# hruffieux/atlasqtl

Measured on NVIDIA B200. Metric: SNPxtrait CAVI updates/s, higher is better.
Workload: dtype f64

## Files before the change

### atlasqtl_b200/_lib.py

```python
import ctypes
import os

import numpy as np

_HERE = os.path.dirname(os.path.abspath(__file__))
LIB_PATH = os.environ.get("AQ_LIB") or os.path.join(_HERE, "libatlasqtl_b200.so")
_DP = ctypes.POINTER(ctypes.c_double)
_IP = ctypes.POINTER(ctypes.c_int32)

EXPORTS = ["aq_last_error", "aq_version", "aq_device_info", "aq_create", "aq_destroy", "aq_dims", "aq_set_order",
           "aq_set_state", "aq_get_state", "aq_get_residual", "aq_refresh_tables", "aq_sweep", "aq_rowsums_zpart",
           "aq_rowsums_zpart_dev", "aq_launch_count", "aq_last_sweep_ms", "aq_last_ms", "aq_sync", "aq_coreDualLoop",
           "aq_set_missing", "aq_set_state_mis", "aq_sweep_mis", "aq_ppi_count_sum", "aq_ppi_next_above", "aq_ppi_collect",
           "aq_prep_x", "aq_prep_geno", "aq_prep_result", "aq_prep_destroy", "aq_prep_launch_count", "aq_create_prepared",
           "aq_get_x", "aq_get_y", "aq_snapshot", "aq_snapshot_fetch", "aq_coreDualMisLoop", "aq_sweep_plan",
           "aq_test_logistic", "aq_prep_dims", "aq_release_x"]


class AtlasqtlB200Error(RuntimeError):
    pass


_lib = None


def load():
    global _lib
    if _lib is not None:
        return _lib
    if not os.path.exists(LIB_PATH):
        raise AtlasqtlB200Error(f"{LIB_PATH} not found: build it with `python -m atlasqtl_b200.build` "
                                "(there is no CPU fallback for the CAVI sweep)")
    lib = ctypes.CDLL(LIB_PATH)
    lib.aq_last_error.restype = ctypes.c_char_p
    lib.aq_launch_count.restype = ctypes.c_int64
    lib.aq_launch_count.argtypes = [ctypes.c_void_p]
    lib.aq_prep_launch_count.restype = ctypes.c_int64
    lib.aq_prep_launch_count.argtypes = [ctypes.c_void_p]
    _lib = lib
    return lib


def check(rc):
    if rc != 0:
        raise AtlasqtlB200Error(f"atlasqtl_b200 error {rc}: {load().aq_last_error().decode()}")


def dptr(a):
    if a is None:
        return None
    assert isinstance(a, np.ndarray) and a.dtype == np.float64
    return a.ctypes.data_as(_DP)


def iptr(a):
    if a is None:
        return None
    assert isinstance(a, np.ndarray) and a.dtype == np.int32 and a.flags.c_contiguous
    return a.ctypes.data_as(_IP)


def fmat(a):
    return np.asfortranarray(a, dtype=np.float64)
```

### atlasqtl_b200/compat.py

```python
import ctypes

import numpy as np

from . import _lib


def coreDualLoop(cp_X, cp_Y_X, gam_vb, log_Phi_theta_plus_zeta, log_1_min_Phi_theta_plus_zeta, log_sig2_inv_vb,
                 log_tau_vb, m1_beta, cp_betaX_X, mu_beta_vb, sig2_beta_vb, tau_vb, shuffled_ind, sample_q, c=1.0,
                 device=0):
    lib = _lib.load()
    p, q = gam_vb.shape
    mats = (cp_X, cp_Y_X, gam_vb, log_Phi_theta_plus_zeta, log_1_min_Phi_theta_plus_zeta, m1_beta, cp_betaX_X, mu_beta_vb)
    for m in mats:
        if not (isinstance(m, np.ndarray) and m.dtype == np.float64 and m.flags.f_contiguous):
            raise TypeError("matrices must be Fortran-ordered float64 arrays (R's double storage)")
    if cp_X.shape != (p, p) or cp_Y_X.shape != (q, p):
        raise ValueError("cp_X must be p x p and cp_Y_X q x p")
    vecs = [np.ascontiguousarray(v, dtype=np.float64) for v in (log_tau_vb, sig2_beta_vb, tau_vb)]
    si = np.ascontiguousarray(shuffled_ind, dtype=np.int32)
    sq = np.ascontiguousarray(sample_q, dtype=np.int32)
    _lib.check(lib.aq_coreDualLoop(ctypes.c_int(device), p, q, _lib.dptr(cp_X), _lib.dptr(cp_Y_X), _lib.dptr(gam_vb),
                                   _lib.dptr(log_Phi_theta_plus_zeta), _lib.dptr(log_1_min_Phi_theta_plus_zeta),
                                   ctypes.c_double(log_sig2_inv_vb), _lib.dptr(vecs[0]), _lib.dptr(m1_beta),
                                   _lib.dptr(cp_betaX_X), _lib.dptr(mu_beta_vb), _lib.dptr(vecs[1]), _lib.dptr(vecs[2]),
                                   _lib.iptr(si), len(si), _lib.iptr(sq), len(sq), ctypes.c_double(c)))


def coreDualMisLoop(cp_X, cp_X_rm, cp_Y_X, gam_vb, log_Phi_theta_plus_zeta, log_1_min_Phi_theta_plus_zeta, log_sig2_inv_vb,
                    log_tau_vb, m1_beta, cp_betaX_X, mu_beta_vb, sig2_beta_vb, tau_vb, shuffled_ind, sample_q, c=1.0,
                    device=0):
    lib = _lib.load()
    p, q = gam_vb.shape
    mats = (cp_X, cp_Y_X, gam_vb, log_Phi_theta_plus_zeta, log_1_min_Phi_theta_plus_zeta, m1_beta, cp_betaX_X, mu_beta_vb,
            sig2_beta_vb) + tuple(cp_X_rm)
    for m in mats:
        if not (isinstance(m, np.ndarray) and m.dtype == np.float64 and m.flags.f_contiguous):
            raise TypeError("matrices must be Fortran-ordered float64 arrays (R's double storage)")
    if cp_X.shape != (p, p) or cp_Y_X.shape != (q, p) or sig2_beta_vb.shape != (p, q):
        raise ValueError("cp_X must be p x p, cp_Y_X q x p and sig2_beta_vb p x q")
    if len(cp_X_rm) != q or any(m.shape != (p, p) for m in cp_X_rm):
        raise ValueError("cp_X_rm must be a list of q p x p matrices")
    vecs = [np.ascontiguousarray(v, dtype=np.float64) for v in (log_tau_vb, tau_vb)]
    si = np.ascontiguousarray(shuffled_ind, dtype=np.int32)
    sq = np.ascontiguousarray(sample_q, dtype=np.int32)
    rm = (_lib._DP * q)(*[_lib.dptr(m) for m in cp_X_rm])
    _lib.check(lib.aq_coreDualMisLoop(ctypes.c_int(device), p, q, _lib.dptr(cp_X), rm, _lib.dptr(cp_Y_X), _lib.dptr(gam_vb),
                                      _lib.dptr(log_Phi_theta_plus_zeta), _lib.dptr(log_1_min_Phi_theta_plus_zeta),
                                      ctypes.c_double(log_sig2_inv_vb), _lib.dptr(vecs[0]), _lib.dptr(m1_beta),
                                      _lib.dptr(cp_betaX_X), _lib.dptr(mu_beta_vb), _lib.dptr(sig2_beta_vb),
                                      _lib.dptr(vecs[1]), _lib.iptr(si), len(si), _lib.iptr(sq), len(sq),
                                      ctypes.c_double(c)))


def logistic_neg_device(x, device=0, variant=0):
    lib = _lib.load()
    x = np.ascontiguousarray(x, dtype=np.float64)
    out = np.empty_like(x)
    _lib.check(lib.aq_test_logistic(ctypes.c_int(device), ctypes.c_int(variant), _lib.dptr(x), _lib.dptr(out),
                                    ctypes.c_int(x.size)))
    return out
```

### atlasqtl_b200/csrc/aq_api.cu

```cuda
#include <algorithm>
#include <cmath>
#include <cstdio>
#include <cstdlib>
#include <cstring>
#include <numeric>
#include <string>
#include <vector>

#include "../../include/atlasqtl_b200.h"
#include "aq_internal.h"
#include "aq_mis.cuh"
#include "aq_prep.cuh"
#include "aq_select.cuh"
#include "aq_stream.cuh"
#include "aq_sweep.cuh"

using namespace aq;

namespace {

thread_local std::string g_err;

int fail(int code, const std::string& msg) {
    g_err = msg;
// ... 536 lines not shown
    if (c->stream) cudaStreamSynchronize(c->stream);
    double* bufs[] = {c->xraw, c->xtiles, c->ymat, c->resid, c->gam, c->mu, c->dtab, c->wtab, c->i0tab, c->tvec,
                      c->ovec, c->theta, c->zeta, c->rowsum, c->partials, c->scalar, c->stage};
    for (double* b : bufs)
        if (b) cudaFree(b);
    if (c->order_dev) cudaFree(c->order_dev);
    if (c->seg_done) cudaFree(c->seg_done);
    if (c->mask) cudaFree(c->mask);
    if (c->mbits) cudaFree(c->mbits);
    if (c->mis_off_dev) cudaFree(c->mis_off_dev);
    if (c->mis_idx_dev) cudaFree(c->mis_idx_dev);
    for (double* b : {c->gk, c->atab, c->ltab})
        if (b) cudaFree(b);
    if (c->copy_stream) cudaStreamSynchronize(c->copy_stream);
    for (double* b : {c->sig2tab, c->xnsq, c->n_obs, c->mis_out, c->sel_partial, c->rowpart, c->snap_gam, c->snap_mu, c->stage2})
        if (b) cudaFree(b);
    if (c->ev0) cudaEventDestroy(c->ev0);
    if (c->ev1) cudaEventDestroy(c->ev1);
    for (cudaEvent_t e : {c->evr0, c->evr1, c->evt0, c->evt1})
        if (e) cudaEventDestroy(e);
    if (c->ev_snap) cudaEventDestroy(c->ev_snap);
    if (c->copy_stream) cudaStreamDestroy(c->copy_stream);
    if (c->stream) cudaStreamDestroy(c->stream);
    delete c;
    return AQ_OK;
}

}

namespace {
int create_impl(aq_ctx** out, int device, int n, int p, int q_local, const double* X, const aq_prep* prep, const double* Y,
                double* n_obs) {
    if (n < 2 || p < 1 || q_local < 1) return fail(AQ_EINVAL, "aq_create: need n >= 2, p >= 1, q >= 1");
    int sm = 0;
    int rc = aq_device_info(device, &sm, nullptr, nullptr);
    if (rc != AQ_OK) return rc;
    CfgInfo cfg;
    if (!pick_cfg(n, q_local, sm, &cfg))
        return fail(AQ_EUNSUPPORTED, "aq_create: n > 7168 is beyond the 8-CTA sample-split cluster kernel");
    aq_ctx* c = new aq_ctx();
    c->device = device;
    c->n = n;
    c->p = p;
    c->q = q_local;
    c->cfg = cfg;
    c->sm_count = sm;
    c->p_pad = (p + kBlk - 1) / kBlk * kBlk;
    c->q_pad = (q_local + 95) / 96 * 96;
    c->nb = c->p_pad / kBlk;
    c->ld_resid = cfg.n_pad * cfg.ncta;
    c->ntiles = (q_local + cfg.kT - 1) / cfg.kT;
    const size_t pq = (size_t)c->p_pad * c->q_pad;
    c->stage_cols = (int)std::max<size_t>(1, std::min<size_t>((size_t)q_local, ((size_t)256 << 20) / (sizeof(double) * (size_t)p)));
    c->n_partials = (size_t)((c->q + 255) / 256) * ((c->p + kTabRowsPerBlock - 1) / kTabRowsPerBlock);
#define AQ_ALLOC(ptr, count)                                                              \
    do {                                                                                  \
        cudaError_t e_ = cudaMalloc((void**)&(ptr), sizeof(*(ptr)) * (size_t)(count));    \
        if (e_ != cudaSuccess) {                                                          \
            cudaGetLastError();                                                           \
            aq_destroy(c);                                                                \
            return fail(AQ_ENOMEM, std::string("cudaMalloc ") + #ptr + ": " + cudaGetErrorString(e_)); \
        }                                                                                 \
    } while (0)
    AQ_ALLOC(c->xraw, (size_t)n * p);
    AQ_ALLOC(c->xtiles, (size_t)c->nb * cfg.ncta * cfg.tile_doubles);
    AQ_ALLOC(c->ymat, (size_t)c->q_pad * c->ld_resid);
    AQ_ALLOC(c->resid, (size_t)c->q_pad * c->ld_resid);
    AQ_ALLOC(c->gam, pq);
    AQ_ALLOC(c->mu, pq);
    AQ_ALLOC(c->dtab, pq);
    AQ_ALLOC(c->wtab, pq);
    AQ_ALLOC(c->i0tab, pq);
    AQ_ALLOC(c->tvec, 3 * (size_t)c->q_pad);
    AQ_ALLOC(c->ovec, 5 * (size_t)c->q_pad);
    AQ_ALLOC(c->theta, c->p_pad);
    AQ_ALLOC(c->zeta, c->q_pad);
    AQ_ALLOC(c->rowsum, c->p_pad);
    AQ_ALLOC(c->partials, c->n_partials);
    AQ_ALLOC(c->scalar, 8);
    AQ_ALLOC(c->stage, (size_t)c->stage_cols * p);
    AQ_ALLOC(c->order_dev, c->p_pad);
#undef AQ_ALLOC
    cudaError_t e = cudaStreamCreateWithFlags(&c->stream, cudaStreamNonBlocking);
    if (e == cudaSuccess) e = cudaEventCreate(&c->ev0);
    if (e == cudaSuccess) e = cudaEventCreate(&c->ev1);
    if (e == cudaSuccess) e = cudaEventCreate(&c->evr0);
    if (e == cudaSuccess) e = cudaEventCreate(&c->evr1);
    if (e == cudaSuccess) e = cudaEventCreate(&c->evt0);
    if (e == cudaSuccess) e = cudaEventCreate(&c->evt1);
    if (e == cudaSuccess) e = cudaMemsetAsync(c->ymat, 0, sizeof(double) * (size_t)c->q_pad * c->ld_resid, c->stream);
    if (e == cudaSuccess) e = cudaMemsetAsync(c->gam, 0, sizeof(double) * pq, c->stream);
    if (e == cudaSuccess) e = cudaMemsetAsync(c->mu, 0, sizeof(double) * pq, c->stream);
    if (e == cudaSuccess) e = cudaMemsetAsync(c->dtab, 0, sizeof(double) * pq, c->stream);
    if (e == cudaSuccess) e = cudaMemsetAsync(c->wtab, 0, sizeof(double) * pq, c->stream);
    if (e == cudaSuccess) e = cudaMemsetAsync(c->i0tab, 0, sizeof(double) * pq, c->stream);
    if (e == cudaSuccess) e = cudaMemsetAsync(c->ovec, 0, sizeof(double) * 5 * (size_t)c->q_pad, c->stream);
    if (e == cudaSuccess) e = cudaMemsetAsync(c->rowsum, 0, sizeof(double) * c->p_pad, c->stream);
    if (e == cudaSuccess && X) e = cudaMemcpyAsync(c->xraw, X, sizeof(double) * (size_t)n * p, cudaMemcpyHostToDevice, c->stream);
    if (e == cudaSuccess && prep) {
        if (prep->geno)
            materialise_kernel<<<p, 256, 0, c->stream>>>(SrcGeno{prep->gd, prep->bytes_per_col}, n, prep->st, prep->kept_dev, p, c->xraw);
        else
            materialise_kernel<<<p, 256, 0, c->stream>>>(SrcDouble{prep->xd, n}, n, prep->st, prep->kept_dev, p, c->xraw);
        e = cudaGetLastError();
        c->launches++;
    }
    if (e == cudaSuccess)
// ... 336 lines not shown
}

int aq_snapshot(aq_ctx* c) {
    if (!c) return fail(AQ_EINVAL, "NULL context");
    if (!c->have_state) return fail(AQ_ESTATE, "aq_snapshot before aq_set_state");
    AQ_CUDA(cudaSetDevice(c->device));
    const size_t pq = (size_t)c->p_pad * c->q_pad;
    if (!c->snap_gam) AQ_CUDA(cudaMalloc((void**)&c->snap_gam, sizeof(double) * pq));
    if (!c->snap_mu) AQ_CUDA(cudaMalloc((void**)&c->snap_mu, sizeof(double) * pq));
    if (!c->stage2) AQ_CUDA(cudaMalloc((void**)&c->stage2, sizeof(double) * (size_t)c->stage_cols * c->p));
    if (!c->ev_snap) AQ_CUDA(cudaEventCreateWithFlags(&c->ev_snap, cudaEventDisableTiming));
    if (!c->copy_stream) AQ_CUDA(cudaStreamCreateWithFlags(&c->copy_stream, cudaStreamNonBlocking));
    AQ_CUDA(cudaStreamSynchronize(c->copy_stream));
    AQ_CUDA(cudaMemcpyAsync(c->snap_gam, c->gam, sizeof(double) * pq, cudaMemcpyDeviceToDevice, c->stream));
    AQ_CUDA(cudaMemcpyAsync(c->snap_mu, c->mu, sizeof(double) * pq, cudaMemcpyDeviceToDevice, c->stream));
    AQ_CUDA(cudaEventRecord(c->ev_snap, c->stream));
    c->have_snap = true;
    return AQ_OK;
}

int aq_snapshot_fetch(aq_ctx* c, double* gam_vb, double* mu_beta_vb, double* beta_vb) {
    if (!c) return fail(AQ_EINVAL, "NULL context");
    if (!c->have_snap) return fail(AQ_ESTATE, "aq_snapshot_fetch before aq_snapshot");
    AQ_CUDA(cudaSetDevice(c->device));
    AQ_CUDA(cudaStreamWaitEvent(c->copy_stream, c->ev_snap, 0));
    double* outs[3] = {gam_vb, mu_beta_vb, beta_vb};
    for (int which = 0; which < 3; ++which) {
        if (!outs[which]) continue;
        const double* a = which == 1 ? c->snap_mu : c->snap_gam;
        const double* b = which == 2 ? c->snap_mu : nullptr;
        for (int k0 = 0; k0 < c->q; k0 += c->stage_cols) {
            const int kc = std::min(c->stage_cols, c->q - k0);
            dim3 grid((c->p + 31) / 32, (kc + 31) / 32), block(32, 8);
            dev_to_cm_kernel<<<grid, block, 0, c->copy_stream>>>(a, b, which == 2 ? 1 : 0, c->p, kc, k0, c->q_pad, c->stage2);
            AQ_CUDA(cudaGetLastError());
            AQ_CUDA(cudaMemcpyAsync(outs[which] + (size_t)k0 * c->p, c->stage2, sizeof(double) * (size_t)kc * c->p,
                                    cudaMemcpyDeviceToHost, c->copy_stream));
            AQ_CUDA(cudaStreamSynchronize(c->copy_stream));
        }
    }
    return AQ_OK;
}

int aq_get_residual(aq_ctx* c, double* resid) {
    if (!c || !resid) return fail(AQ_EINVAL, "NULL argument");
    if (!c->have_state) return fail(AQ_ESTATE, "aq_get_residual before aq_set_state");
    AQ_CUDA(cudaSetDevice(c->device));
    AQ_CUDA(cudaMemcpy2DAsync(resid, sizeof(double) * c->n, c->resid, sizeof(double) * c->ld_resid, sizeof(double) * c->n,
                              c->q, cudaMemcpyDeviceToHost, c->stream));
    AQ_CUDA(cudaStreamSynchronize(c->stream));
    return AQ_OK;
}

int aq_refresh_tables(aq_ctx* c, const double* theta_vb, const double* zeta_vb, double c_next, double* elbo_b_part) {
    if (!c || !theta_vb || !zeta_vb) return fail(AQ_EINVAL, "aq_refresh_tables: NULL argument");
    if (!(c_next > 0.0)) return fail(AQ_EINVAL, "aq_refresh_tables: c_next must be positive");
    if (elbo_b_part && !c->have_state) return fail(AQ_ESTATE, "aq_refresh_tables: ELBO part needs a state");
    AQ_CUDA(cudaSetDevice(c->device));
    c->rowpart_rows = 0;
    AQ_CUDA(cudaMemcpyAsync(c->theta, theta_vb, sizeof(double) * c->p, cudaMemcpyHostToDevice, c->stream));
    AQ_CUDA(cudaMemcpyAsync(c->zeta, zeta_vb, sizeof(double) * c->q, cudaMemcpyHostToDevice, c->stream));
    const int c_is_one = std::fabs(c_next - 1.0) < 1.5e-8;
    dim3 grid((c->q + 255) / 256, (c->p + kTabRowsPerBlock - 1) / kTabRowsPerBlock);
    AQ_CUDA(cudaEventRecord(c->evt0, c->stream));
    tables_kernel<<<grid, 256, 0, c->stream>>>(c->theta, c->zeta, c->p, c->q, c->q_pad, c_is_one ? 1.0 : std::sqrt(c_next),
                                               c_is_one, c->gam, c->dtab, c->wtab, c->i0tab, elbo_b_part ? 1 : 0,
                                               c->partials);
    AQ_CUDA(cudaGetLastError());
    c->launches++;
    if (elbo_b_part) {
        sum_partials_kernel<<<1, 1024, 0, c->stream>>>(c->partials, c->n_partials, c->scalar);
        AQ_CUDA(cudaGetLastError());
        c->launches++;
        AQ_CUDA(cudaMemcpyAsync(elbo_b_part, c->scalar, sizeof(double), cudaMemcpyDeviceToHost, c->stream));
    }
    AQ_CUDA(cudaEventRecord(c->evt1, c->stream));
    AQ_CUDA(cudaStreamSynchronize(c->stream));
    AQ_CUDA(cudaEventElapsedTime(&c->last_tables_ms, c->evt0, c->evt1));
    c->have_tables = true;
    return AQ_OK;
}

int aq_sweep(aq_ctx* c, double cc, double log_sig2_inv_vb, const double* tau_vb, const double* log_tau_vb,
             const double* sig2_beta_vb, double* colsum_gam, double* colsum_gam_mu2, double* colsum_beta2,
             double* resid_sq, double* colsum_zpart) {
    if (!c || !tau_vb || !log_tau_vb || !sig2_beta_vb) return fail(AQ_EINVAL, "aq_sweep: NULL argument");
    if (c->has_mis) return fail(AQ_ESTATE, "aq_sweep: this context has missing responses, use aq_sweep_mis");
    if (!c->have_state) return fail(AQ_ESTATE, "aq_sweep before aq_set_state");
    if (!c->have_tables) return fail(AQ_ESTATE, "aq_sweep before aq_refresh_tables");
    if (!(cc > 0.0)) return fail(AQ_EINVAL, "aq_sweep: c must be positive");
    AQ_CUDA(cudaSetDevice(c->device));
    AQ_CUDA(cudaMemcpyAsync(c->tvec, tau_vb, sizeof(double) * c->q, cudaMemcpyHostToDevice, c->stream));
    AQ_CUDA(cudaMemcpyAsync(c->tvec + c->q_pad, log_tau_vb, sizeof(double) * c->q, cudaMemcpyHostToDevice, c->stream));
    AQ_CUDA(cudaMemcpyAsync(c->tvec + 2 * (size_t)c->q_pad, sig2_beta_vb, sizeof(double) * c->q, cudaMemcpyHostToDevice,
                            c->stream));
    int rc = launch_sweep(c, 0, cc, log_sig2_inv_vb);
    if (rc != AQ_OK) return rc;
    rc = fetch_outputs(c, colsum_gam, colsum_gam_mu2, colsum_beta2, resid_sq, colsum_zpart);
    if (rc != AQ_OK) return rc;
    AQ_CUDA(cudaStreamSynchronize(c->stream));
    AQ_CUDA(cudaEventElapsedTime(&c->last_ms, c->ev0, c->ev1));
    return AQ_OK;
}

int aq_rowsums_zpart_dev(aq_ctx* c, double** rowsum_zpart_dev) {
    if (!c || !rowsum_zpart_dev) return fail(AQ_EINVAL, "NULL argument");
    if (!c->have_state || !c->have_tables) return fail(AQ_ESTATE, "aq_rowsums_zpart before state/tables");
    AQ_CUDA(cudaSetDevice(c->device));
    AQ_CUDA(cudaEventRecord(c->evr0, c->stream));
    if (c->rowpart_rows > 0) {
        int rows = c->rowpart_rows;
        if (c->rowpart_k_tail >= 0) {
            const int kt = c->rowpart_k_tail;
            rowsums_kernel<<<(c->p + 7) / 8, 256, 0, c->stream>>>(c->gam + kt, c->wtab + kt, c->i0tab + kt, c->p, c->q - kt,
                                                                  c->q_pad, c->rowpart + (size_t)rows * c->p_pad);
            AQ_CUDA(cudaGetLastError());
            c->launches++;
            ++rows;
        }
        rowpart_reduce_kernel<<<(c->p + 31) / 32, dim3(32, 8), 0, c->stream>>>(c->rowpart, rows, c->p, c->p_pad, c->rowsum);
// ... 329 lines not shown
    if (e == cudaSuccess && ncopy) e = cudaMemcpy(out_gam, dg, sizeof(double) * ncopy, cudaMemcpyDeviceToHost);
    cudaFree(dj);
    cudaFree(dk);
    cudaFree(dg);
    if (e != cudaSuccess) {
        cudaGetLastError();
        return fail(e == cudaErrorMemoryAllocation ? AQ_ENOMEM : AQ_ECUDA, std::string("aq_ppi_collect: ") + cudaGetErrorString(e));
    }
    *n_found = (int64_t)found;
    return AQ_OK;
}

int64_t aq_launch_count(const aq_ctx* c) { return c ? c->launches : 0; }

int aq_sweep_plan(const aq_ctx* c, int* traits_per_tile, int* ntiles, int* groups, int* nseg) {
    if (!c) return fail(AQ_EINVAL, "NULL context");
    if (traits_per_tile) *traits_per_tile = c->cfg.kT;
    if (ntiles) *ntiles = c->ntiles;
    if (groups) *groups = c->max_groups[0];
    if (nseg) *nseg = c->last_nseg;
    return AQ_OK;
}

namespace {
__global__ void test_logistic_kernel(const double* __restrict__ x, double* __restrict__ out, int n, int variant) {
    const int i = blockIdx.x * blockDim.x + threadIdx.x;
    if (i < n) out[i] = variant ? aq::logistic_neg<true>(x[i]) : aq::logistic_neg<false>(x[i]);
}
}

int aq_test_logistic(int device, int variant, const double* x, double* out, int n) {
    if (!x || !out || n < 0 || (variant != 0 && variant != 1)) return fail(AQ_EINVAL, "aq_test_logistic: bad argument");
    if (n == 0) return AQ_OK;
    int rc = aq_device_info(device, nullptr, nullptr, nullptr);
    if (rc != AQ_OK) return rc;
    double *dx = nullptr, *dout = nullptr;
    AQ_CUDA(cudaMalloc((void**)&dx, sizeof(double) * (size_t)n));
    cudaError_t e = cudaMalloc((void**)&dout, sizeof(double) * (size_t)n);
    if (e == cudaSuccess) e = cudaMemcpy(dx, x, sizeof(double) * (size_t)n, cudaMemcpyHostToDevice);
    if (e == cudaSuccess) {
        test_logistic_kernel<<<(n + 255) / 256, 256>>>(dx, dout, n, variant);
        e = cudaGetLastError();
    }
    if (e == cudaSuccess) e = cudaMemcpy(out, dout, sizeof(double) * (size_t)n, cudaMemcpyDeviceToHost);
    cudaFree(dx);
    if (dout) cudaFree(dout);
    if (e != cudaSuccess) {
        cudaGetLastError();
        return fail(AQ_ECUDA, std::string("aq_test_logistic: ") + cudaGetErrorString(e));
    }
    return AQ_OK;
}

int aq_last_sweep_ms(const aq_ctx* c, float* ms) {
    if (!c || !ms) return fail(AQ_EINVAL, "NULL argument");
    *ms = c->last_ms;
    return AQ_OK;
}

int aq_last_ms(const aq_ctx* c, int which, float* ms) {
    if (!c || !ms) return fail(AQ_EINVAL, "NULL argument");
    if (which == 0) *ms = c->last_ms;
    else if (which == 1) *ms = c->last_rows_ms;
    else if (which == 2) *ms = c->last_tables_ms;
    else return fail(AQ_EINVAL, "aq_last_ms: which must be 0 (sweep), 1 (row sums) or 2 (tables)");
    return AQ_OK;
}

int aq_sync(aq_ctx* c) {
    if (!c) return fail(AQ_EINVAL, "NULL context");
    AQ_CUDA(cudaSetDevice(c->device));
    AQ_CUDA(cudaStreamSynchronize(c->stream));
    return AQ_OK;
}

}
```

### atlasqtl_b200/csrc/aq_stream.cuh

```cuda
#pragma once
#include "aq_common.cuh"

namespace aq {

__global__ void build_tiles_kernel(const double* __restrict__ xraw, const int* __restrict__ order, int n, int p,
                                   int xs, int n_pad_c, size_t tile_stride, double* __restrict__ tiles) {
    const int b = blockIdx.x, r = blockIdx.y, nslice = gridDim.y;
    double* tile = tiles + ((size_t)b * nslice + r) * tile_stride;
    for (int t = 0; t < kBlk; ++t) {
        const int pos = b * kBlk + t;
        const int j = pos < p ? order[pos] : -1;
        for (int i = threadIdx.x; i < xs; i += blockDim.x) {
            const int li = swz(i, t);
            const int gi = r * n_pad_c + li;
            tile[t * xs + i] = (j >= 0 && li < n_pad_c && gi < n) ? xraw[(size_t)j * n + gi] : 0.0;
        }
        if (threadIdx.x == 0) reinterpret_cast<int*>(tile + kBlk * xs + 128)[t] = j;
    }
    if (threadIdx.x < 8) reinterpret_cast<int*>(tile + kBlk * xs + 128)[8 + threadIdx.x] = 0;
}

__global__ void gram_band_kernel(double* __restrict__ tiles, int n_pad_c, int nslice, int xs, size_t tile_stride) {
    const int b = blockIdx.x;
    const int t = threadIdx.x >> 4, u = threadIdx.x & 15;
    double acc = 0.0;
    if (u >= 8 || b + 1 < (int)gridDim.x) {
        const int uu = u & 7;
        const int bo = (u >= 8) ? b : b + 1;
        for (int r = 0; r < nslice; ++r) {
            const double* xt = tiles + ((size_t)b * nslice + r) * tile_stride + t * xs;
            const double* xu = tiles + ((size_t)bo * nslice + r) * tile_stride + uu * xs;
            for (int i = 0; i < n_pad_c; ++i) acc = fma(xt[swz(i, t)], xu[swz(i, uu)], acc);
        }
    }
    for (int r = 0; r < nslice; ++r) tiles[((size_t)b * nslice + r) * tile_stride + kBlk * xs + t * 16 + u] = acc;
}

__global__ void cm_to_dev_kernel(const double* __restrict__ src, int p, int kc, int k_first, int q_pad,
                                 double* __restrict__ dst) {
    __shared__ double tile[32][33];
    const int j0 = blockIdx.x * 32, c0 = blockIdx.y * 32;
    for (int r = threadIdx.y; r < 32; r += blockDim.y) {
        const int kk = c0 + r, j = j0 + threadIdx.x;
        tile[r][threadIdx.x] = (kk < kc && j < p) ? src[(size_t)kk * p + j] : 0.0;
    }
    __syncthreads();
    for (int r = threadIdx.y; r < 32; r += blockDim.y) {
        const int j = j0 + r, kk = c0 + threadIdx.x;
        if (j < p && kk < kc) dst[(size_t)j * q_pad + k_first + kk] = tile[threadIdx.x][r];
    }
}
__global__ void dev_to_cm_kernel(const double* __restrict__ a, const double* __restrict__ b2, int op, int p, int kc,
                                 int k_first, int q_pad, double* __restrict__ dst) {
    __shared__ double tile[32][33];
    const int j0 = blockIdx.x * 32, c0 = blockIdx.y * 32;
    for (int r = threadIdx.y; r < 32; r += blockDim.y) {
        const int j = j0 + r, kk = c0 + threadIdx.x;
        double v = 0.0;
        if (j < p && kk < kc) {
            const size_t off = (size_t)j * q_pad + k_first + kk;
            v = a[off];
            if (op == 1) v *= b2[off];
        }
        tile[r][threadIdx.x] = v;
    }
    __syncthreads();
    for (int r = threadIdx.y; r < 32; r += blockDim.y) {
        const int kk = c0 + r, j = j0 + threadIdx.x;
        if (kk < kc && j < p) dst[(size_t)kk * p + j] = tile[threadIdx.x][r];
    }
}

__global__ void fill_kernel(double* __restrict__ x, size_t nelem, double v) {
    for (size_t i = blockIdx.x * (size_t)blockDim.x + threadIdx.x; i < nelem; i += (size_t)gridDim.x * blockDim.x) x[i] = v;
}

constexpr int kTabRowsPerBlock = 8;

__device__ __forceinline__ double fast_rcp(double d) {
    double y;
    asm("rcp.approx.ftz.f64 %0, %1;" : "=d"(y) : "d"(d));
    const double e0 = fma(-d, y, 1.0);
    return fma(y, fma(e0, e0, e0), y);
}

struct NormalPoint {
    double log_tail, log_body;
    double r_tail, r_body;
};
__device__ __forceinline__ NormalPoint normal_point(double u, bool want_logs, bool want_ratios) {
    const double kRs2 = 0.70710678118654752440, kSqrt2OverPi = 0.79788456080286535588, kInvSqrt2Pi = 0.39894228040143267794;
    NormalPoint o;
    const double a = fabs(u) * kRs2;
    const double E = erfcx(a);
    const double e2 = exp(-0.5 * u * u);
    const double Q = 0.5 * E * e2;
    if (want_logs) {
        o.log_tail = log(0.5 * E) - 0.5 * u * u;
        o.log_body = log1p(-Q);
    }
    if (want_ratios) {
        o.r_tail = kSqrt2OverPi * fast_rcp(E);
        o.r_body = kInvSqrt2Pi * e2 * fast_rcp(1.0 - Q);
    }
    return o;
}

__device__ __forceinline__ double normal_point_logodds(double u, bool want_ratios, double& r_tail, double& r_body) {
    const double kRs2 = 0.70710678118654752440, kSqrt2OverPi = 0.79788456080286535588, kInvSqrt2Pi = 0.39894228040143267794;
    const double a = fabs(u) * kRs2;
    const double E = erfcx(a);
    const double e2 = exp(-0.5 * u * u);
    const double Q = 0.5 * E * e2;
    const double inv = fast_rcp(1.0 - Q);
    if (want_ratios) {
        r_tail = kSqrt2OverPi * fast_rcp(E);
        r_body = kInvSqrt2Pi * e2 * inv;
    }
    return log(0.5 * E * inv) - 0.5 * u * u;
}

__global__ void __launch_bounds__(256) tables_kernel(const double* __restrict__ theta, const double* __restrict__ zeta, int p,
                                                     int q, int q_pad, double sqrt_c, int c_is_one,
                                                     const double* __restrict__ gam, double* __restrict__ dtab,
                                                     double* __restrict__ wtab, double* __restrict__ i0tab, int want_elbo,
                                                     double* __restrict__ partials) {
    const double eps = 1.8189894035458565e-12;
    const int k = blockIdx.x * blockDim.x + threadIdx.x;
    double part = 0.0;
    if (k < q) {
        const double zk = zeta[k];
        const int j0 = blockIdx.y * kTabRowsPerBlock;
#pragma unroll 1
        for (int r = 0; r < kTabRowsPerBlock; ++r) {
            const int j = j0 + r;
            if (j >= p) break;
            const size_t off = (size_t)j * q_pad + k;
            const double u = theta[j] + zk;
            double lp = 0.0, lq = 0.0, U = u, r_tail = 0.0, r_body = 0.0;
            if (want_elbo) {
                const NormalPoint nu = normal_point(u, true, c_is_one != 0);
                lp = (u >= 0.0) ? nu.log_body : nu.log_tail;
                lq = (u >= 0.0) ? nu.log_tail : nu.log_body;
                dtab[off] = lq - lp;
                r_tail = nu.r_tail;
                r_body = nu.r_body;
            } else {
                const double lo = normal_point_logodds(u, c_is_one != 0, r_tail, r_body);
                dtab[off] = (u >= 0.0) ? lo : -lo;
            }
            if (!c_is_one) {
                U = sqrt_c * u;
                const NormalPoint nU = normal_point(U, false, true);
                r_tail = nU.r_tail;
                r_body = nU.r_body;
            }
            double m1 = (U >= 0.0) ? r_body : r_tail;
            double m0 = -((U >= 0.0) ? r_tail : r_body);
            if (m1 < -U) m1 = -U;
            if (m0 > -U) m0 = -U;
            wtab[off] = m1 - m0;
            i0tab[off] = m0;
            if (want_elbo) {
                const double gm = gam[off];
                part += gm * lp + (1.0 - gm) * lq - gm * log(gm + eps) - (1.0 - gm) * log(1.0 - gm + eps);
            }
        }
    }
    if (want_elbo) {
        __shared__ double red[8];
        part = warp_sum(part);
        if ((threadIdx.x & 31) == 0) red[threadIdx.x >> 5] = part;
        __syncthreads();
        if (threadIdx.x == 0) {
            double s = 0.0;
            for (int w = 0; w < 8; ++w) s += red[w];
            partials[(size_t)blockIdx.y * gridDim.x + blockIdx.x] = s;
        }
    }
}

__global__ void sum_partials_kernel(const double* __restrict__ x, size_t n, double* __restrict__ out) {
    __shared__ double red[32];
    double s = 0.0;
    for (size_t i = threadIdx.x; i < n; i += blockDim.x) s += x[i];
    s = warp_sum(s);
    if ((threadIdx.x & 31) == 0) red[threadIdx.x >> 5] = s;
    __syncthreads();
    if (threadIdx.x < 32) {
        double v = threadIdx.x < (blockDim.x >> 5) ? red[threadIdx.x] : 0.0;
        v = warp_sum(v);
        if (threadIdx.x == 0) *out = v;
    }
}

__global__ void __launch_bounds__(256) rowsums_kernel(const double* __restrict__ gam, const double* __restrict__ wtab,
                                                      const double* __restrict__ i0tab, int p, int q, int q_pad,
                                                      double* __restrict__ rowsum) {
    const int j = blockIdx.x * (blockDim.x >> 5) + (threadIdx.x >> 5);
    if (j >= p) return;
    const int lane = threadIdx.x & 31;
    const size_t base = (size_t)j * q_pad;
    double s0 = 0.0, s1 = 0.0;
    const int q2 = q & ~1;
    for (int k = 2 * lane; k < q2; k += 64) {
        const double2 g = *reinterpret_cast<const double2*>(gam + base + k);
        const double2 w = *reinterpret_cast<const double2*>(wtab + base + k);
        const double2 i0 = *reinterpret_cast<const double2*>(i0tab + base + k);
        s0 += fma(g.x, w.x, i0.x);
        s1 += fma(g.y, w.y, i0.y);
    }
    if (lane == 0 && q2 < q) s0 += fma(gam[base + q2], wtab[base + q2], i0tab[base + q2]);
    const double s = warp_sum(s0 + s1);
    if (lane == 0) rowsum[j] = s;
}

__global__ void __launch_bounds__(256) rowpart_reduce_kernel(const double* __restrict__ rowpart, int nrows, int p, int p_pad,
                                                             double* __restrict__ rowsum) {
    __shared__ double red[8][33];
    const int j = blockIdx.x * 32 + threadIdx.x;
    double s0 = 0.0, s1 = 0.0, s2 = 0.0, s3 = 0.0;
    if (j < p) {
        const double* col = rowpart + j;
        int r = threadIdx.y;
        for (; r + 24 < nrows; r += 32) {
            s0 += col[(size_t)r * p_pad];
            s1 += col[(size_t)(r + 8) * p_pad];
            s2 += col[(size_t)(r + 16) * p_pad];
            s3 += col[(size_t)(r + 24) * p_pad];
// ... 15 lines not shown
```

### include/atlasqtl_b200.h

```cpp
#ifndef ATLASQTL_B200_H_
#define ATLASQTL_B200_H_

#include <stdint.h>

#ifdef __cplusplus
extern "C" {
#endif

#define AQ_OK 0
#define AQ_EINVAL (-1)
#define AQ_ECUDA (-2)
#define AQ_ENOMEM (-3)
#define AQ_ESTATE (-4)
#define AQ_EUNSUPPORTED (-5)

typedef struct aq_ctx aq_ctx;

const char* aq_last_error(void);
int aq_version(void);

int aq_device_info(int device, int* sm_count, int64_t* free_bytes, int64_t* total_bytes);

int aq_create(aq_ctx** out, int device, int n, int p, int q_local, const double* X, const double* Y);
int aq_destroy(aq_ctx* ctx);
// ... 23 lines not shown
int aq_snapshot_fetch(aq_ctx* ctx, double* gam_vb, double* mu_beta_vb, double* beta_vb);

int aq_get_residual(aq_ctx* ctx, double* resid);

int aq_refresh_tables(aq_ctx* ctx, const double* theta_vb, const double* zeta_vb, double c_next,
                      double* elbo_b_part);

int aq_sweep(aq_ctx* ctx, double c, double log_sig2_inv_vb, const double* tau_vb, const double* log_tau_vb,
             const double* sig2_beta_vb, double* colsum_gam, double* colsum_gam_mu2, double* colsum_beta2,
             double* resid_sq, double* colsum_zpart);

int aq_rowsums_zpart(aq_ctx* ctx, double* rowsum_zpart);
int aq_rowsums_zpart_dev(aq_ctx* ctx, double** rowsum_zpart_dev);

int aq_set_missing(aq_ctx* ctx, const double* mis_pat, double* n_obs);
int aq_set_state_mis(aq_ctx* ctx, const double* gam_vb, const double* mu_beta_vb, double* colsum_gam,
                     double* colsum_gam_mu2, double* colsum_beta2, double* resid_sq, double* colsum_xn_gam,
                     double* colsum_xn_gam_mu2, double* colsum_xn_beta2);
int aq_sweep_mis(aq_ctx* ctx, double c, double log_sig2_inv_vb, double sig2_inv_vb, const double* tau_vb,
                 const double* log_tau_vb, double* colsum_gam, double* colsum_gam_mu2, double* colsum_sig2b_gam,
                 double* colsum_xn_gam_mu2, double* colsum_xn_sig2b_gam, double* colsum_xn_beta2, double* resid_sq,
                 double* colsum_zpart, double* colsum_gam_logsig2b);

int aq_ppi_count_sum(aq_ctx* ctx, double t, double* count, double* sum);
int aq_ppi_next_above(aq_ctx* ctx, double t, double* next);
int aq_ppi_collect(aq_ctx* ctx, int mode, double lo, double hi, int64_t capacity, int32_t* out_j, int32_t* out_k,
                   double* out_gam, int64_t* n_found);

int64_t aq_launch_count(const aq_ctx* ctx);

int aq_last_sweep_ms(const aq_ctx* ctx, float* ms);
int aq_last_ms(const aq_ctx* ctx, int which, float* ms);

int aq_sync(aq_ctx* ctx);

int aq_coreDualLoop(int device, int p, int q, const double* cp_X, const double* cp_Y_X, double* gam_vb,
                    const double* log_Phi_theta_plus_zeta, const double* log_1_min_Phi_theta_plus_zeta,
                    double log_sig2_inv_vb, const double* log_tau_vb, double* m1_beta, double* cp_betaX_X,
                    double* mu_beta_vb, const double* sig2_beta_vb, const double* tau_vb,
                    const int32_t* shuffled_ind, int n_ind, const int32_t* sample_q, int n_q, double c);


int aq_coreDualMisLoop(int device, int p, int q, const double* cp_X, const double* const* cp_X_rm, const double* cp_Y_X,
                       double* gam_vb, const double* log_Phi_theta_plus_zeta,
                       const double* log_1_min_Phi_theta_plus_zeta, double log_sig2_inv_vb, const double* log_tau_vb,
                       double* m1_beta, double* cp_betaX_X, double* mu_beta_vb, const double* sig2_beta_vb,
                       const double* tau_vb, const int32_t* shuffled_ind, int n_ind, const int32_t* sample_q, int n_q,
                       double c);

int aq_sweep_plan(const aq_ctx* ctx, int* traits_per_tile, int* ntiles, int* groups, int* nseg);

int aq_test_logistic(int device, int variant, const double* x, double* out, int n);

#ifdef __cplusplus
}
#endif
#endif
```

Baseline: 6.398 billion.

## Rewrite normal-table kernel with custom erfcx/exp/log and two traits per thread

Replaces libdevice erfcx/exp/log calls in the per-(SNP,trait) normal-table kernel with inlined polynomial approximations (erfcx on a rational-transformed argument, a Taylor exp, a fdlibm-style log). It also templates the kernel on the anneal and ELBO flags to remove runtime branches, and has each thread handle two adjacent traits with double2 loads and stores. A device test entry point is added to check the new table values against references. The hand-written math risks accuracy loss near edge cases, and the double2 accesses assume q_pad keeps offsets 16-byte aligned.

Result: faster. 6.481 billion (median of 6 runs) (+1.3%).

```diff
diff --git a/atlasqtl_b200/_lib.py b/atlasqtl_b200/_lib.py
--- a/atlasqtl_b200/_lib.py
+++ b/atlasqtl_b200/_lib.py
@@ -14,7 +14,7 @@
            "aq_set_missing", "aq_set_state_mis", "aq_sweep_mis", "aq_ppi_count_sum", "aq_ppi_next_above", "aq_ppi_collect",
            "aq_prep_x", "aq_prep_geno", "aq_prep_result", "aq_prep_destroy", "aq_prep_launch_count", "aq_create_prepared",
            "aq_get_x", "aq_get_y", "aq_snapshot", "aq_snapshot_fetch", "aq_coreDualMisLoop", "aq_sweep_plan",
-           "aq_test_logistic", "aq_prep_dims", "aq_release_x"]
+           "aq_test_logistic", "aq_test_normal_tables", "aq_prep_dims", "aq_release_x"]
 
 
 class AtlasqtlB200Error(RuntimeError):
diff --git a/atlasqtl_b200/compat.py b/atlasqtl_b200/compat.py
--- a/atlasqtl_b200/compat.py
+++ b/atlasqtl_b200/compat.py
@@ -59,3 +59,16 @@
     _lib.check(lib.aq_test_logistic(ctypes.c_int(device), ctypes.c_int(variant), _lib.dptr(x), _lib.dptr(out),
                                     ctypes.c_int(x.size)))
     return out
+
+
+def normal_tables_device(u, c=1.0, gam=None, device=0):
+    lib = _lib.load()
+    u = np.ascontiguousarray(u, dtype=np.float64)
+    want_elbo = gam is not None
+    g = np.ascontiguousarray(np.broadcast_to(gam, u.shape), dtype=np.float64) if want_elbo else None
+    out = np.empty((4 if want_elbo else 3, u.size))
+    _lib.check(lib.aq_test_normal_tables(ctypes.c_int(device), _lib.dptr(u.ravel()), ctypes.c_int(u.size),
+                                         ctypes.c_double(c), ctypes.c_int(int(want_elbo)),
+                                         _lib.dptr(g.ravel()) if want_elbo else None, _lib.dptr(out)))
+    names = ["d", "w", "i0", "elbo_b"]
+    return {names[i]: out[i].reshape(u.shape) for i in range(out.shape[0])}
diff --git a/atlasqtl_b200/csrc/aq_api.cu b/atlasqtl_b200/csrc/aq_api.cu
--- a/atlasqtl_b200/csrc/aq_api.cu
+++ b/atlasqtl_b200/csrc/aq_api.cu
@@ -612,7 +612,7 @@
     c->ntiles = (q_local + cfg.kT - 1) / cfg.kT;
     const size_t pq = (size_t)c->p_pad * c->q_pad;
     c->stage_cols = (int)std::max<size_t>(1, std::min<size_t>((size_t)q_local, ((size_t)256 << 20) / (sizeof(double) * (size_t)p)));
-    c->n_partials = (size_t)((c->q + 255) / 256) * ((c->p + kTabRowsPerBlock - 1) / kTabRowsPerBlock);
+    c->n_partials = (size_t)((c->q + kTabTraitsPerBlock - 1) / kTabTraitsPerBlock) * ((c->p + kTabRowsPerBlock - 1) / kTabRowsPerBlock);
 #define AQ_ALLOC(ptr, count)                                                              \
     do {                                                                                  \
         cudaError_t e_ = cudaMalloc((void**)&(ptr), sizeof(*(ptr)) * (size_t)(count));    \
@@ -1055,6 +1055,15 @@
     return AQ_OK;
 }
 
+static bool tables_anneal(double c_next) { return !(std::fabs(c_next - 1.0) < 1.5e-8); }
+static double tables_sqrt_c(double c_next) { return tables_anneal(c_next) ? std::sqrt(c_next) : 1.0; }
+using TablesKernel = void (*)(const double*, const double*, int, int, int, double, const double*, double*, double*, double*,
+                              double*);
+static TablesKernel tables_kernel_for(double c_next, bool want_elbo) {
+    if (tables_anneal(c_next)) return want_elbo ? tables_kernel<true, true> : tables_kernel<true, false>;
+    return want_elbo ? tables_kernel<false, true> : tables_kernel<false, false>;
+}
+
 int aq_refresh_tables(aq_ctx* c, const double* theta_vb, const double* zeta_vb, double c_next, double* elbo_b_part) {
     if (!c || !theta_vb || !zeta_vb) return fail(AQ_EINVAL, "aq_refresh_tables: NULL argument");
     if (!(c_next > 0.0)) return fail(AQ_EINVAL, "aq_refresh_tables: c_next must be positive");
@@ -1063,12 +1072,11 @@
     c->rowpart_rows = 0;
     AQ_CUDA(cudaMemcpyAsync(c->theta, theta_vb, sizeof(double) * c->p, cudaMemcpyHostToDevice, c->stream));
     AQ_CUDA(cudaMemcpyAsync(c->zeta, zeta_vb, sizeof(double) * c->q, cudaMemcpyHostToDevice, c->stream));
-    const int c_is_one = std::fabs(c_next - 1.0) < 1.5e-8;
-    dim3 grid((c->q + 255) / 256, (c->p + kTabRowsPerBlock - 1) / kTabRowsPerBlock);
+    dim3 grid((c->q + kTabTraitsPerBlock - 1) / kTabTraitsPerBlock, (c->p + kTabRowsPerBlock - 1) / kTabRowsPerBlock);
     AQ_CUDA(cudaEventRecord(c->evt0, c->stream));
-    tables_kernel<<<grid, 256, 0, c->stream>>>(c->theta, c->zeta, c->p, c->q, c->q_pad, c_is_one ? 1.0 : std::sqrt(c_next),
-                                               c_is_one, c->gam, c->dtab, c->wtab, c->i0tab, elbo_b_part ? 1 : 0,
-                                               c->partials);
+    const auto kernel = tables_kernel_for(c_next, elbo_b_part != nullptr);
+    kernel<<<grid, kTabThreads, 0, c->stream>>>(c->theta, c->zeta, c->p, c->q, c->q_pad, tables_sqrt_c(c_next), c->gam,
+                                                c->dtab, c->wtab, c->i0tab, c->partials);
     AQ_CUDA(cudaGetLastError());
     c->launches++;
     if (elbo_b_part) {
@@ -1504,6 +1512,58 @@
     return AQ_OK;
 }
 
+extern "C++" {
+namespace {
+template <bool kAnneal, bool kElbo>
+__global__ void test_tables_kernel(const double* __restrict__ u, const double* __restrict__ gam, int n, double sqrt_c,
+                                   double* __restrict__ out) {
+    const int i = blockIdx.x * blockDim.x + threadIdx.x;
+    if (i >= n) return;
+    const aq::TableEntry e = aq::table_entry<kAnneal, kElbo>(u[i], sqrt_c);
+    out[i] = e.d;
+    out[(size_t)n + i] = e.w;
+    out[2 * (size_t)n + i] = e.i0;
+    if (kElbo) out[3 * (size_t)n + i] = aq::elbo_b_term(gam[i], e.lp, e.lq);
+}
+}
+}
+
+int aq_test_normal_tables(int device, const double* u, int n, double c, int want_elbo, const double* gam, double* out) {
+    if (!u || !out || n < 0 || !(c > 0.0) || (want_elbo && !gam)) return fail(AQ_EINVAL, "aq_test_normal_tables: bad argument");
+    if (n == 0) return AQ_OK;
+    int rc = aq_device_info(device, nullptr, nullptr, nullptr);
+    if (rc != AQ_OK) return rc;
+    const size_t nout = (want_elbo ? 4 : 3) * (size_t)n;
+    double *du = nullptr, *dg = nullptr, *dout = nullptr;
+    cudaError_t e = cudaMalloc((void**)&du, sizeof(double) * 2 * (size_t)n);
+    if (e == cudaSuccess) {
+        dg = du + n;
+        e = cudaMalloc((void**)&dout, sizeof(double) * nout);
+    }
+    if (e == cudaSuccess) e = cudaMemcpy(du, u, sizeof(double) * (size_t)n, cudaMemcpyHostToDevice);
+    if (e == cudaSuccess && want_elbo) e = cudaMemcpy(dg, gam, sizeof(double) * (size_t)n, cudaMemcpyHostToDevice);
+    if (e == cudaSuccess) {
+        const double sc = tables_sqrt_c(c);
+        const unsigned nb = (unsigned)((n + 255) / 256);
+        if (tables_anneal(c)) {
+            if (want_elbo) test_tables_kernel<true, true><<<nb, 256>>>(du, dg, n, sc, dout);
+            else test_tables_kernel<true, false><<<nb, 256>>>(du, dg, n, sc, dout);
+        } else {
+            if (want_elbo) test_tables_kernel<false, true><<<nb, 256>>>(du, dg, n, sc, dout);
+            else test_tables_kernel<false, false><<<nb, 256>>>(du, dg, n, sc, dout);
+        }
+        e = cudaGetLastError();
+    }
+    if (e == cudaSuccess) e = cudaMemcpy(out, dout, sizeof(double) * nout, cudaMemcpyDeviceToHost);
+    if (du) cudaFree(du);
+    if (dout) cudaFree(dout);
+    if (e != cudaSuccess) {
+        cudaGetLastError();
+        return fail(AQ_ECUDA, std::string("aq_test_normal_tables: ") + cudaGetErrorString(e));
+    }
+    return AQ_OK;
+}
+
 int aq_last_sweep_ms(const aq_ctx* c, float* ms) {
     if (!c || !ms) return fail(AQ_EINVAL, "NULL argument");
     *ms = c->last_ms;
diff --git a/atlasqtl_b200/csrc/aq_stream.cuh b/atlasqtl_b200/csrc/aq_stream.cuh
--- a/atlasqtl_b200/csrc/aq_stream.cuh
+++ b/atlasqtl_b200/csrc/aq_stream.cuh
@@ -76,6 +76,8 @@
 }
 
 constexpr int kTabRowsPerBlock = 8;
+constexpr int kTabThreads = 256;
+constexpr int kTabTraitsPerBlock = 2 * kTabThreads;
 
 __device__ __forceinline__ double fast_rcp(double d) {
     double y;
@@ -84,97 +86,173 @@
     return fma(y, fma(e0, e0, e0), y);
 }
 
-struct NormalPoint {
-    double log_tail, log_body;
-    double r_tail, r_body;
+template <int N>
+__device__ __forceinline__ double horner(const double (&c)[N], double x) {
+    double acc = c[0];
+#pragma unroll
+    for (int i = 1; i < N; ++i) acc = fma(acc, x, c[i]);
+    return acc;
+}
+
+__device__ constexpr double kErfcxP[25] = {
+    8.86421901642709157e-10, 9.88579883113936507e-10, -8.50039792977261530e-09,
+    -1.33263648130038336e-08, 4.18078469884558215e-08, 1.01870006000728852e-07,
+    -1.41600649402659871e-07, -6.16649607760435273e-07, 3.56838391539922039e-07,
+    3.47241460287568619e-06, -7.31510516415906236e-07, -2.01005679312892271e-05,
+    4.94948499257059483e-06, 1.25099352355631071e-04, -1.05159799815011774e-04,
+    -7.79832272108399124e-04, 1.88869035915615528e-03, 2.52939181606623908e-03,
+    -2.37705149186458881e-02, 6.83080273439784780e-02, -1.19273663415306985e-01,
+    1.29645158702760610e-01, -4.75622943534508708e-02, -1.35621106124581170e-01,
+    1.25300805826972961e+00};
+__device__ constexpr double kLogR[7] = {
+    1.46164496850434061e-01, 1.53317216005560419e-01, 1.81828891252617225e-01,
+    2.22222111347950807e-01, 2.85714286259754868e-01, 3.99999999998995048e-01,
+    6.66666666666666963e-01};
+
+__device__ __forceinline__ double erfcx_nonneg(double a) {
+    const double t = (a - 3.0) * fast_rcp(a + 3.0);
+    return horner(kErfcxP, t) * fast_rcp(fma(2.0, a, 1.0));
+}
+
+__device__ constexpr double kInvFact[13] = {1.0, 1.0, 1.0 / 2, 1.0 / 6, 1.0 / 24, 1.0 / 120, 1.0 / 720, 1.0 / 5040,
+                                            1.0 / 40320, 1.0 / 362880, 1.0 / 3628800, 1.0 / 39916800, 1.0 / 479001600};
+__device__ __forceinline__ double exp_nonpos(double x) {
+    const double kInvLn2 = 1.4426950408889634074, kMagic = 6755399441055744.0;
+    const double t = fma(x, kInvLn2, kMagic);
+    const double k = t - kMagic;
+    double r = fma(-k, 6.93147180369123816490e-01, x);
+    r = fma(-k, 1.90821492927058770002e-10, r);
+    const int ki = __double2loint(t);
+    const int k1 = ki >> 1;
+    const double s1 = __hiloint2double((k1 + 1023) << 20, 0);
+    const double s2 = __hiloint2double((ki - k1 + 1023) << 20, 0);
+    double e = 1.0 / 6227020800.0;
+#pragma unroll
+    for (int i = 12; i >= 0; --i) e = fma(e, r, kInvFact[i]);
+    return (e * s1) * s2;
+}
+
+__device__ __forceinline__ double log1p_reduced(double f) {
+    const double s = f * fast_rcp(2.0 + f);
+    const double z = s * s;
+    return fma(-s, fma(-z, horner(kLogR, z), f), f);
+}
+constexpr double kLn2Hi = 6.93147180369123816490e-01, kLn2Lo = 1.90821492927058770002e-10;
+
+__device__ __forceinline__ double log_pos(double x) {
+    int hx = __double2hiint(x) + (0x3ff00000 - 0x3fe6a09e);
+    const int k = (hx >> 20) - 0x3ff;
+    hx = (hx & 0x000fffff) + 0x3fe6a09e;
+    const double f = __hiloint2double(hx, __double2loint(x)) - 1.0;
+    const double kd = __hiloint2double(0x43300000, k + 0x80000000) - 4503601774854144.0;
+    return fma(kd, kLn2Hi, fma(kd, kLn2Lo, log1p_reduced(f)));
+}
+
+__device__ __forceinline__ double log1m(double Q) {
+    const bool big = Q > 0.29289321881345248;
+    const double l = log1p_reduced(big ? fma(-2.0, Q, 1.0) : -Q);
+    return big ? l - 0.69314718055994530942 : l;
+}
+
+struct NormalCore {
+    double E, e2, Q, rbody;
+    double hi;
 };
-__device__ __forceinline__ NormalPoint normal_point(double u, bool want_logs, bool want_ratios) {
-    const double kRs2 = 0.70710678118654752440, kSqrt2OverPi = 0.79788456080286535588, kInvSqrt2Pi = 0.39894228040143267794;
-    NormalPoint o;
-    const double a = fabs(u) * kRs2;
-    const double E = erfcx(a);
-    const double e2 = exp(-0.5 * u * u);
-    const double Q = 0.5 * E * e2;
-    if (want_logs) {
-        o.log_tail = log(0.5 * E) - 0.5 * u * u;
-        o.log_body = log1p(-Q);
-    }
-    if (want_ratios) {
-        o.r_tail = kSqrt2OverPi * fast_rcp(E);
-        o.r_body = kInvSqrt2Pi * e2 * fast_rcp(1.0 - Q);
-    }
+__device__ __forceinline__ NormalCore normal_core(double u) {
+    const double kRs2 = 0.70710678118654752440;
+    NormalCore o;
+    o.hi = u * u;
+    const double lo = fma(u, u, -o.hi);
+    double a = fabs(u) * kRs2;
+    a = a > 1e300 ? 1e300 : a;
+    o.E = erfcx_nonneg(a);
+    const double e = exp_nonpos(-0.5 * o.hi);
+    o.e2 = o.hi > 1492.0 ? 0.0 : fma(e, -0.5 * lo, e);
+    o.Q = 0.5 * o.E * o.e2;
+    o.rbody = fast_rcp(1.0 - o.Q);
     return o;
 }
 
-__device__ __forceinline__ double normal_point_logodds(double u, bool want_ratios, double& r_tail, double& r_body) {
-    const double kRs2 = 0.70710678118654752440, kSqrt2OverPi = 0.79788456080286535588, kInvSqrt2Pi = 0.39894228040143267794;
-    const double a = fabs(u) * kRs2;
-    const double E = erfcx(a);
-    const double e2 = exp(-0.5 * u * u);
-    const double Q = 0.5 * E * e2;
-    const double inv = fast_rcp(1.0 - Q);
-    if (want_ratios) {
-        r_tail = kSqrt2OverPi * fast_rcp(E);
-        r_body = kInvSqrt2Pi * e2 * inv;
-    }
-    return log(0.5 * E * inv) - 0.5 * u * u;
-}
-
-__global__ void __launch_bounds__(256) tables_kernel(const double* __restrict__ theta, const double* __restrict__ zeta, int p,
-                                                     int q, int q_pad, double sqrt_c, int c_is_one,
-                                                     const double* __restrict__ gam, double* __restrict__ dtab,
-                                                     double* __restrict__ wtab, double* __restrict__ i0tab, int want_elbo,
-                                                     double* __restrict__ partials) {
+struct TableEntry {
+    double d, w, i0;
+    double lp, lq;
+};
+template <bool kAnneal, bool kElbo>
+__device__ __forceinline__ TableEntry table_entry(double u, double sqrt_c) {
+    const double kSqrt2OverPi = 0.79788456080286535588, kInvSqrt2Pi = 0.39894228040143267794;
+    TableEntry o;
+    const NormalCore nu = normal_core(u);
+    const double lodds = fma(-0.5, nu.hi, log_pos(0.5 * nu.E * nu.rbody));
+    o.d = (u >= 0.0) ? lodds : -lodds;
+    if constexpr (kElbo) {
+        const double lbody = log1m(nu.Q), ltail = lodds + lbody;
+        o.lp = (u >= 0.0) ? lbody : ltail;
+        o.lq = (u >= 0.0) ? ltail : lbody;
+    }
+    double U = u;
+    NormalCore nU = nu;
+    if constexpr (kAnneal) {
+        U = sqrt_c * u;
+        nU = normal_core(U);
+    }
+    const double r_tail = kSqrt2OverPi * fast_rcp(nU.E);
+    const double r_body = kInvSqrt2Pi * nU.e2 * nU.rbody;
+    const double m1 = fmax((U >= 0.0) ? r_body : r_tail, -U);
+    const double m0 = fmin(-((U >= 0.0) ? r_tail : r_body), -U);
+    o.w = m1 - m0;
+    o.i0 = m0;
+    return o;
+}
+
+__device__ __forceinline__ double elbo_b_term(double gm, double lp, double lq) {
     const double eps = 1.8189894035458565e-12;
-    const int k = blockIdx.x * blockDim.x + threadIdx.x;
+    return gm * lp + (1.0 - gm) * lq - gm * log_pos(gm + eps) - (1.0 - gm) * log_pos(1.0 - gm + eps);
+}
+
+template <bool kAnneal, bool kElbo>
+__global__ void __launch_bounds__(kTabThreads) tables_kernel(const double* __restrict__ theta, const double* __restrict__ zeta,
+                                                            int p, int q, int q_pad, double sqrt_c,
+                                                            const double* __restrict__ gam, double* __restrict__ dtab,
+                                                            double* __restrict__ wtab, double* __restrict__ i0tab,
+                                                            double* __restrict__ partials) {
+    const int k = 2 * (blockIdx.x * blockDim.x + threadIdx.x);
     double part = 0.0;
     if (k < q) {
-        const double zk = zeta[k];
+        const bool both = k + 1 < q;
+        const double2 z = *reinterpret_cast<const double2*>(zeta + k);
         const int j0 = blockIdx.y * kTabRowsPerBlock;
 #pragma unroll 1
         for (int r = 0; r < kTabRowsPerBlock; ++r) {
             const int j = j0 + r;
             if (j >= p) break;
             const size_t off = (size_t)j * q_pad + k;
-            const double u = theta[j] + zk;
-            double lp = 0.0, lq = 0.0, U = u, r_tail = 0.0, r_body = 0.0;
-            if (want_elbo) {
-                const NormalPoint nu = normal_point(u, true, c_is_one != 0);
-                lp = (u >= 0.0) ? nu.log_body : nu.log_tail;
-                lq = (u >= 0.0) ? nu.log_tail : nu.log_body;
-                dtab[off] = lq - lp;
-                r_tail = nu.r_tail;
-                r_body = nu.r_body;
+            const double th = theta[j];
+            const TableEntry a = table_entry<kAnneal, kElbo>(th + z.x, sqrt_c);
+            const TableEntry b = table_entry<kAnneal, kElbo>(th + z.y, sqrt_c);
+            if (both) {
+                *reinterpret_cast<double2*>(dtab + off) = make_double2(a.d, b.d);
+                *reinterpret_cast<double2*>(wtab + off) = make_double2(a.w, b.w);
+                *reinterpret_cast<double2*>(i0tab + off) = make_double2(a.i0, b.i0);
             } else {
-                const double lo = normal_point_logodds(u, c_is_one != 0, r_tail, r_body);
-                dtab[off] = (u >= 0.0) ? lo : -lo;
+                dtab[off] = a.d;
+                wtab[off] = a.w;
+                i0tab[off] = a.i0;
             }
-            if (!c_is_one) {
-                U = sqrt_c * u;
-                const NormalPoint nU = normal_point(U, false, true);
-                r_tail = nU.r_tail;
-                r_body = nU.r_body;
+            if constexpr (kElbo) {
+                const double2 g = *reinterpret_cast<const double2*>(gam + off);
+                part += elbo_b_term(g.x, a.lp, a.lq);
+                if (both) part += elbo_b_term(g.y, b.lp, b.lq);
             }
-            double m1 = (U >= 0.0) ? r_body : r_tail;
-            double m0 = -((U >= 0.0) ? r_tail : r_body);
-            if (m1 < -U) m1 = -U;
-            if (m0 > -U) m0 = -U;
-            wtab[off] = m1 - m0;
-            i0tab[off] = m0;
-            if (want_elbo) {
-                const double gm = gam[off];
-                part += gm * lp + (1.0 - gm) * lq - gm * log(gm + eps) - (1.0 - gm) * log(1.0 - gm + eps);
-            }
-        }
-    }
-    if (want_elbo) {
-        __shared__ double red[8];
+        }
+    }
+    if constexpr (kElbo) {
+        __shared__ double red[kTabThreads / 32];
         part = warp_sum(part);
         if ((threadIdx.x & 31) == 0) red[threadIdx.x >> 5] = part;
         __syncthreads();
         if (threadIdx.x == 0) {
             double s = 0.0;
-            for (int w = 0; w < 8; ++w) s += red[w];
+            for (int w = 0; w < kTabThreads / 32; ++w) s += red[w];
             partials[(size_t)blockIdx.y * gridDim.x + blockIdx.x] = s;
         }
     }
diff --git a/include/atlasqtl_b200.h b/include/atlasqtl_b200.h
--- a/include/atlasqtl_b200.h
+++ b/include/atlasqtl_b200.h
@@ -99,6 +99,8 @@
 
 int aq_test_logistic(int device, int variant, const double* x, double* out, int n);
 
+int aq_test_normal_tables(int device, const double* u, int n, double c, int want_elbo, const double* gam, double* out);
+
 #ifdef __cplusplus
 }
 #endif
```
